# illini-robomaster/irmv_detection

Measured on AMD Instinct MI355X. Metric: end-to-end FPS (preprocess→NMS→PnP) 640×640 YOLOv8n, 1/2/4/8 MI355X, higher is better.
Workload: dtype f16

## Files before the change

### irmv_detection_amd/csrc/engine.cpp

```cpp
#include "engine_internal.hpp"

static thread_local std::string g_err;
int irmv::fail(int code, const std::string &msg) { g_err = msg; return code; }

extern "C" const char *irmv_last_error(void) { return g_err.c_str(); }
extern "C" const char *irmv_version(void)
{
    static char buf[96];
    static std::once_flag once;
    std::call_once(once, [] {
        int v = 0;
        if (hipRuntimeGetVersion(&v) != hipSuccess) v = 0;
        snprintf(buf, sizeof buf, "irmv_hip 0.3 (gfx950; HIP runtime %d)", v);
    });
    return buf;
}
extern "C" int irmv_device_synchronize(int device)
{
    HIP_TRY(hipSetDevice(device));
    HIP_TRY(hipDeviceSynchronize());
    return IRMV_OK;
}
extern "C" int irmv_device_count(int *count)
{
// ... 199 lines not shown
    cfg->bayer_gain_q8[0] = cfg->bayer_gain_q8[1] = cfg->bayer_gain_q8[2] = 256;
}

static EngineSwitches read_switches()
{
    auto set = [](const char *name) { return getenv(name) != nullptr; };
    auto starts = [](const char *name, char c) { const char *v = getenv(name); return v && v[0] == c; };
    auto off = [&](const char *name) { return starts(name, '0'); };
    auto is1 = [&](const char *name) { return starts(name, '1'); };
    EngineSwitches s;
    TuneSwitches &t = s.tune;
    t.untuned = off("IRMV_AUTOTUNE"); t.verbose = set("IRMV_AUTOTUNE_VERBOSE"); t.warn = set("IRMV_TUNE_WARN");
    const char *s2 = getenv("IRMV_FORCE_S2"), *wres = getenv("IRMV_FORCE_WRES");
    t.has_s2 = s2 != nullptr; t.force_s2 = s2 ? s2 : "";
    t.has_wres = wres != nullptr; t.force_wres = wres ? wres : "";
    t.force_pw = set("IRMV_FORCE_PW"); t.force_pwn = set("IRMV_FORCE_PWN"); t.force_cm = set("IRMV_FORCE_CM");
    t.force_w8 = set("IRMV_FORCE_W8"); t.force_nt8 = set("IRMV_FORCE_NT8"); t.force_pf4 = set("IRMV_FORCE_PF4");
    t.no_pw = set("IRMV_NO_PW"); t.no_pwn = set("IRMV_NO_PWN"); t.no_pf2 = set("IRMV_NO_PF2"); t.no_pf4 = set("IRMV_NO_PF4");
    t.no_cm = set("IRMV_NO_CM"); t.no_w8 = set("IRMV_NO_W8"); t.no_nt8 = set("IRMV_NO_NT8"); t.no_wres = set("IRMV_NO_WRES");
    t.no_deep = is1("IRMV_NO_DEEP");
    s.front.fastx = !off("IRMV_FRONT_FASTX"); s.front.direct = !off("IRMV_FRONT_DIRECT"); s.front.tall = !off("IRMV_FRONT_TILE8");
    s.fused_front = !off("IRMV_FUSED_FRONT"); s.fused_c2f = !off("IRMV_FUSED_C2F"); s.bneck64 = !off("IRMV_BNECK64"); s.kpt3 = !off("IRMV_KPT3");
    s.fused_head = !off("IRMV_FUSED_HEAD");
    s.merge_head0 = off("IRMV_MERGE_HEAD0") ? 0 : (is1("IRMV_MERGE_HEAD0") ? 1 : -1);
    s.group_head = !off("IRMV_GROUP_HEAD"); s.group_verbose = set("IRMV_GROUP_VERBOSE"); s.group_force = set("IRMV_GROUP_FORCE");
    if (const char *ns = getenv("IRMV_STREAMS")) { s.has_streams = true; s.streams = atoi(ns); }
    s.numa = !off("IRMV_NUMA");
    s.inline_copies = is1("IRMV_INLINE_COPIES"); s.graph_upload = !off("IRMV_GRAPH_UPLOAD"); s.window_upload = !off("IRMV_WINDOW_UPLOAD");
    if (const char *uk = getenv("IRMV_UPLOAD_KERNEL")) s.upload_kernel_blocks = atoi(uk);
    s.sync_launch = starts("IRMV_SYNC_LAUNCH", 'e') ? 1 : (starts("IRMV_SYNC_LAUNCH", 'g') ? 0 : -1);
    s.split_scan = !off("IRMV_SPLIT_SCAN"); s.emit_scan = !off("IRMV_EMIT_SCAN");
    s.sparse_head = !off("IRMV_SPARSE_HEAD"); s.sparse_branch = !off("IRMV_SPARSE_BRANCH");
    s.sparse_gather = !off("IRMV_SPARSE_GATHER");
    if (const char *gg = getenv("IRMV_SPARSE_GATHER_GRID")) s.gather_grid = atoi(gg);
    s.zero_copy_results = !off("IRMV_ZERO_COPY_RESULTS"); s.post_keys_only = is1("IRMV_POST_KEYS_ONLY");
    s.nms_classwalk = !off("IRMV_NMS_CLASSWALK");
    s.meter_merge = !off("IRMV_METER_MERGE");
    s.nms_prefilter = off("IRMV_NMS_PREFILTER") ? 0 : 1;
    if (const char *pe = getenv("IRMV_NMS_PRE")) { int hi = 0, lo = 0; if (sscanf(pe, "%d,%d", &hi, &lo) == 2 && hi >= 64 && hi <= 512 && lo >= 32 && lo < hi) s.nms_prefilter = hi | (lo << 16); }
    if (const char *st = getenv("IRMV_NMS_STAMPS")) { s.nms_stamps = true; s.nms_stamps_slots = atoi(st); }
    return s;
}

constexpr size_t kCfgSizeV1 = offsetof(irmv_engine_cfg, src_format);
constexpr size_t kCfgSizeV2 = offsetof(irmv_engine_cfg, reserved2);
static_assert(offsetof(irmv_engine_cfg, net_height) < kCfgSizeV2 && kCfgSizeV2 < sizeof(irmv_engine_cfg), "three distinct cfg sizes");
static_assert(offsetof(irmv_engine_cfg, win_width) == offsetof(irmv_engine_cfg, reserved2) + 4 && offsetof(irmv_engine_cfg, win_height) + 2 == sizeof(irmv_engine_cfg),
              "win_width / win_height fill the tail of irmv_engine_cfg");

static irmv_engine_cfg window_view(const irmv_engine_cfg &c)
{
    irmv_engine_cfg v = c;
    if (c.win_width > 0 && c.win_height > 0) { v.src_width = c.win_width; v.src_height = c.win_height; }
    v.win_width = v.win_height = 0;
    return v;
}

int irmv::check_letterbox(const irmv_engine_cfg &c)
{
    int nw, nh;
    scaled_size(c, &nw, &nh);
    if (nw < 1 || nh < 1) return fail(IRMV_ERR_ARG, "letterbox: the scaled frame has no row or no column; use IRMV_RESIZE_STRETCH");
    return IRMV_OK;
}

int irmv::resolve_cfg(const irmv_engine_cfg *cfg_in, irmv_engine_cfg *full)
// ... 668 lines not shown
```

### irmv_detection_amd/csrc/engine_internal.hpp

```cpp
#pragma once
#include <hip/hip_runtime.h>

#include <algorithm>
#include <chrono>
#include <cmath>
#include <cstdio>
#include <cstring>
#include <fstream>
#include <map>
#include <mutex>
#include <set>
#include <memory>
#include <string>
#include <vector>

#include "../../include/irmv_hip.h"
#include "irmv_common.hpp"
#include "numa.hpp"

using namespace irmv;

namespace irmv { int fail(int code, const std::string &msg); }
#define HIP_TRY(expr)                                                                                 \
    do {                                                                                              \
// ... 39 lines not shown
struct DevRange { std::string name; MemTag tag; void *base; size_t bytes; };

struct FrontSwitches { bool fastx = true, direct = true, tall = true; };

struct TuneSwitches {
    bool untuned, verbose, warn;
    bool has_s2, has_wres;
    std::string force_s2, force_wres;
    bool force_pw, force_pwn, force_cm, force_w8, force_nt8, force_pf4;
    bool no_pw, no_pwn, no_pf2, no_pf4, no_cm, no_w8, no_nt8, no_wres, no_deep;
};

struct EngineSwitches {
    TuneSwitches tune{};
    FrontSwitches front;
    bool fused_front = true, fused_c2f = true;
    bool bneck64 = true;
    bool kpt3 = true;
    bool fused_head = true;
    int merge_head0 = -1;
    bool group_head = true;
    bool group_verbose = false;
    bool group_force = false;
    bool has_streams = false; int streams = 0;
    bool numa = true;
    bool inline_copies = false;
    bool graph_upload = true;
    int upload_kernel_blocks = 256;
    bool window_upload = true;
    int sync_launch = -1;
    bool split_scan = true;
    bool emit_scan = true, sparse_head = true, sparse_branch = true;
    bool sparse_gather = true;
    int gather_grid = 0;
    bool zero_copy_results = true;
    bool post_keys_only = false;
    bool nms_classwalk = true;
    int nms_prefilter = 1;
    bool meter_merge = true;
    bool nms_stamps = false; int nms_stamps_slots = 0;
};

enum OpKind { OP_PRE, OP_CONV0, OP_CONV, OP_POOL, OP_NMS, OP_LIGHT, OP_FRONT, OP_C2F2, OP_C2F32, OP_DW, OP_SHUF, OP_SCAN, OP_BNECK, OP_KPT3, OP_BOXG, OP_DEMOSAIC, OP_CROP, OP_METER, OP_YAW, OP_PATCH, OP_NUMBER };

struct Op {
    OpKind kind;
    std::string layer;
    ConvCfg cfg{};
    ConvCfg cfg_one{};
    char kname_one[48] = {0};
    SegRef s0, s1;
    int Hin = 0, Win = 0, Hout = 0, Wout = 0, cin = 0, cout = 0, cout_pad = 0, ksteps = 0;
    int out_t = -1, out_coff = 0, res_t = -1, res_coff = 0;
    half_t *w_packed = nullptr;
    half_t *w_k16 = nullptr;
    half_t *w_lds[4] = {nullptr, nullptr, nullptr, nullptr};
    float *bias = nullptr;
    double flops = 0, bytes = 0;
    double w_bytes = 0;
    double out_bytes = 0;
    bool pair = false;
    int level = -1;
    char kname[48] = {0};
    int sub[4] = {-1, -1, -1, -1};
    int mode = 0;
    bool shortcut = false;
    int fuse_next = -1;
    bool fused_away = false;
    int group = -1;
    int bneck = -1;
    int kpt3 = -1;
    int boxg = -1;
    bool gated_first = false;
    int tune_fuse[2] = {-1, -1};
};

enum StepKind { STEP_BATCH, STEP_ONE, STEP_MATERIALIZE, STEP_POST };

struct Launch {
    int op = -1, group = -1;
    bool cfg_one = false;
    bool fused = false;
    unsigned scan = 0;
    bool keys_only = false;
    bool sparse = false;
    int gate = 0;
    bool cand_list = false;
    bool once = false;
    std::string name, layer;
    double flops = 0, bytes = 0, launch_bytes = 0;
};

struct Step {
    StepKind kind;
    int first, count;
    int tile_frame = -1;
    bool crop_pinned = false;
    bool tiled() const { return tile_frame >= 0; }
    bool dev_records() const { return tiled(); }
    int bayer_first() const { return tiled() ? tile_frame : first; }
    int bayer_count() const { return tiled() ? 1 : count; }
    bool operator<(const Step &o) const { return std::tie(first, count, kind, tile_frame, crop_pinned) < std::tie(o.first, o.count, o.kind, o.tile_frame, o.crop_pinned); }
};

struct GraphKey {
    Step step;
    bool upload;
    int view;
    bool operator<(const GraphKey &o) const { return std::tie(upload, view, step) < std::tie(o.upload, o.view, o.step); }
};

enum UploadForm {
    UP_NONE,
    UP_PINNED_CROP,
    UP_KERNEL,
    UP_COPY,
    UP_BANDS,
};
struct Upload { UploadForm form = UP_NONE; int first = 0, count = 0; };

// ... 255 lines not shown
```

### irmv_detection_amd/csrc/engine_plan.cpp

```cpp
#include "engine_internal.hpp"

static bool is_cls_final_carrier(const Op &op) { return op.fuse_next >= 0 && op.level >= 0 && op.layer.rfind("model.22.cv3.", 0) == 0; }

void irmv::finalize_head_fusion(irmv_engine *e)
{
    for (Op &op : e->ops) {
        if (op.fuse_next < 0) continue;
        const bool k16 = op.cfg.cin16 && !op.cfg.lds && !op.cfg_one.lds && !op.cfg.deep && !op.cfg_one.deep && op.cfg.nt == 1 && op.cfg_one.nt == 1 && e->ops[op.fuse_next].w_k16;
        const bool ok = k16 || (op.cfg.lds && op.cfg.nt == 4 && op.cfg_one.lds && op.cfg_one.nt == 4);
        if (!ok) { op.fuse_next = -1; continue; }
        e->ops[op.fuse_next].fused_away = true;
        e->lazy_tensors.insert(e->tensors[op.out_t].name);
        const size_t l = strlen(op.kname), l1 = strlen(op.kname_one);
        snprintf(op.kname + l, sizeof op.kname - l, "+1x1");
        snprintf(op.kname_one + l1, sizeof op.kname_one - l1, "+1x1");
    }
    int fused = 0;
    for (const Op &op : e->ops) fused += is_cls_final_carrier(op);
    e->emit_scan = e->sw.split_scan && fused == 3 && e->sw.emit_scan;
    e->sparse_head = e->emit_scan && e->cand_bits && e->sw.sparse_head;
    e->sparse_branch = e->sparse_head && e->sw.sparse_branch;
}

static bool is_box_final_carrier(const Op &op) { return op.fuse_next >= 0 && op.level >= 0 && op.layer.rfind("model.22.cv2.", 0) == 0; }

static void sparse_head_plan(irmv_engine *e, std::vector<Launch> &plan)
{
    int last_cls = -1;
    bool lvl_cls[3] = {false, false, false};
    for (size_t i = 0; i < plan.size(); i++)
        if (plan[i].scan && plan[i].group < 0) { last_cls = (int)i; lvl_cls[e->ops[plan[i].op].level] = true; }
    auto box_carrier = [&](const Launch &l) {
        const Op &op = e->ops[l.op];
        return l.group < 0 && l.fused && op.kind == OP_CONV && is_box_final_carrier(op) && op.level < 3 && lvl_cls[op.level];
    };
    std::vector<char> first_conv(plan.size(), 0);
    if (e->sparse_branch)
        for (size_t i = 0; i < plan.size(); i++) {
            const Launch &f = plan[i];
            const Op &fo = e->ops[f.op];
            if (f.group >= 0 || f.fused || f.scan || fo.kind != OP_CONV || !(f.cfg_one ? fo.cfg_one : fo.cfg).wr || fo.res_t >= 0) continue;
            int carrier = -1;
            for (size_t j = i + 1; j < plan.size(); j++) {
                const Op &co = e->ops[plan[j].op];
                if (box_carrier(plan[j]) && co.level == fo.level && co.s0.t == fo.out_t && co.s1.C == 0 && co.s0.coff == fo.out_coff && co.Hin == fo.Hout && co.Win == fo.Wout) carrier = plan[j].op;
            }
            bool other = false;
            for (int k = 0; k < (int)e->ops.size(); k++) {
                const Op &o = e->ops[k];
                if (k == carrier || k == f.op) continue;
                other = other || o.s0.t == fo.out_t || o.s1.t == fo.out_t || o.res_t == fo.out_t || o.out_t == fo.out_t;
            }
            first_conv[i] = carrier >= 0 && !other;
        }
    std::vector<Launch> out, moved;
    bool listed = false;
    for (size_t i = 0; i < plan.size(); i++) {
        Launch &l = plan[i];
        Op &op = e->ops[l.op];
        const bool boxg = op.kind == OP_BOXG;
        if (boxg) {
            l.sparse = true;
            l.cand_list = !listed;
            listed = true;
        }
        if (l.scan) {
            if (l.group < 0) l.bytes -= e->ops[op.fuse_next].out_bytes;
            else for (size_t m = 0; m < e->head_groups[l.group].members.size(); m++)
                if (l.scan >> m & 1u) l.bytes -= e->ops[e->ops[e->head_groups[l.group].members[m]].fuse_next].out_bytes;
        }
        const bool cls_first = op.level >= 0 && op.level < 3 && lvl_cls[op.level];
        const bool box = box_carrier(l);
        const bool kpt = op.kind == OP_KPT3 && cls_first && (int)i > last_cls;
        if (box || kpt) {
            l.sparse = true;
            l.bytes -= box ? e->ops[op.fuse_next].out_bytes : op.out_bytes;
            if (e->sparse_branch) l.gate = 1;
        }
        if (first_conv[i]) {
            l.gate = 2;
            op.gated_first = true;
            e->lazy_tensors.insert(e->tensors[op.out_t].name);
        }
        if ((box || first_conv[i] || boxg) && (int)i < last_cls) moved.push_back(l); else out.push_back(l);
        if ((int)i == last_cls) { out.insert(out.end(), moved.begin(), moved.end()); moved.clear(); }
    }
    plan.swap(out);
}

static bool box_gathers(const irmv_engine *e, const Op &g, bool one)
// ... 122 lines not shown
```

### irmv_detection_amd/csrc/engine_step.cpp

```cpp
#include "engine_internal.hpp"

void irmv::fill_conv_args(const irmv_engine *e, const Op &op, int first, int count, ConvArgs &a, bool fused)
{
    a = ConvArgs{};
    auto seg = [&](const SegRef &s) {
        ConvSeg cs{nullptr, 0, 0, 0};
        if (s.t < 0 || s.C == 0) return cs;
        const Tensor &t = e->tensors[s.t];
        cs.p = static_cast<const half_t *>(t.slot(first)) + s.coff;
        cs.ld = t.C;
        cs.C = s.C;
        cs.shift = s.shift;
        return cs;
    };
    a.s0 = seg(op.s0);
    a.s1 = seg(op.s1);
    a.Hin = op.Hin; a.Win = op.Win; a.Hout = op.Hout; a.Wout = op.Wout;
    a.M = count * op.Hout * op.Wout;
    a.Cin = op.cin;
    a.w = op.w_packed;
    a.bias = op.bias;
    const Tensor &ot = e->tensors[op.out_t];
    a.out = static_cast<char *>(ot.slot(first)) + (size_t)op.out_coff * ot.esize();
    a.out_ld = ot.C;
// ... 225 lines not shown
}

static Kpt3Args kpt3_args(const irmv_engine *e, const Op &op, const Launch &l, int first, const PostArgs &pa)
{
    const Op &o0 = e->ops[op.sub[0]], &o1 = e->ops[op.sub[1]], &o2 = e->ops[op.sub[2]];
    const Tensor &xt = e->tensors[o0.s0.t], &ht = e->tensors[o2.out_t];
    Kpt3Args a{};
    a.x = static_cast<const half_t *>(xt.slot(first)) + o0.s0.coff; a.x_ld = xt.C;
    a.H = op.Hin; a.W = op.Win;
    a.tiles_x = (op.Win + kKpt3Tile - 1) / kKpt3Tile; a.tiles_y = (op.Hin + kKpt3Tile - 1) / kKpt3Tile;
    a.w1 = o0.w_lds[0]; a.b1 = o0.bias;
    a.w2 = o1.w_packed; a.b2 = o1.bias;
    a.w3 = o2.w_k16; a.b3 = o2.bias;
    a.out = static_cast<float *>(ht.slot(first)) + o2.out_coff; a.out_ld = ht.C;
    if (l.sparse) { a.cand_bits = pa.cand_bits; a.cand_words = pa.cand_words; a.abase = e->lvl_base[op.level]; a.tile_gate = l.gate; }
    return a;
}

static CandListArgs cand_list_args(const irmv_engine *e, int first, const PostArgs &pa)
{
    CandListArgs a{};
    a.cand_bits = pa.cand_bits; a.cand_words = pa.cand_words;
    const size_t S = (size_t)e->cfg.num_slots;
    for (int l = 0; l < 3; l++) { a.abase[l] = e->lvl_base[l]; a.hw[l] = e->lvl_hw[l]; }
    for (const Op &op : e->ops)
        if (op.kind == OP_BOXG) {
            const int l = op.level;
            a.list[l] = e->boxg_list + (size_t)e->lvl_base[l] * S + (size_t)first * e->lvl_hw[l];
            a.count[l] = e->boxg_count + (size_t)l * S + first;
        }
    return a;
}

static BoxGatherArgs boxg_args(const irmv_engine *e, const Op &op, int first, const PostArgs &pa)
{
    const Op &o0 = e->ops[op.sub[0]], &o1 = e->ops[op.sub[1]], &o2 = e->ops[op.sub[2]];
    const Tensor &xt = e->tensors[o0.s0.t], &ht = e->tensors[o2.out_t];
    const CandListArgs c = cand_list_args(e, first, pa);
    BoxGatherArgs a{};
    a.x = static_cast<const half_t *>(xt.slot(first)) + o0.s0.coff; a.x_ld = xt.C;
    a.H = op.Hin; a.W = op.Win;
    a.w0 = o0.w_lds[2]; a.b0 = o0.bias;
    a.w1 = o1.w_lds[2]; a.b1 = o1.bias;
    a.w2 = o2.w_packed; a.b2 = o2.bias;
    a.out = static_cast<float *>(ht.slot(first)) + o2.out_coff; a.out_ld = ht.C;
    a.list = c.list[op.level]; a.count = c.count[op.level];
    return a;
}

static DwArgs dw_args(const irmv_engine *e, const Op &op, int first)
{
    DwArgs a;
    const Tensor &xt = e->tensors[op.s0.t], &ot = e->tensors[op.out_t];
    a.x = static_cast<const half_t *>(xt.slot(first)) + op.s0.coff; a.x_ld = xt.C;
    a.y = static_cast<half_t *>(ot.slot(first)) + op.out_coff; a.y_ld = ot.C;
    a.w = op.w_packed; a.b = op.bias;
    a.Hin = op.Hin; a.Win = op.Win; a.Hout = op.Hout; a.Wout = op.Wout; a.C = op.cout; a.stride = op.cfg.stride;
    return a;
}

static ShufArgs shuf_args(const irmv_engine *e, const Op &op, int first, int count)
{
    ShufArgs a;
    const Tensor &at = e->tensors[op.s0.t], &bt = e->tensors[op.s1.t], &ot = e->tensors[op.out_t];
    a.a = static_cast<const half_t *>(at.slot(first)) + op.s0.coff; a.a_ld = at.C;
    a.b = static_cast<const half_t *>(bt.slot(first)) + op.s1.coff; a.b_ld = bt.C;
    a.out = static_cast<half_t *>(ot.slot(first)); a.out_ld = ot.C;
    a.bc = op.s0.C;
    a.pixels = (size_t)count * op.Hin * op.Win;
    return a;
}

static Conv0Args conv0_args(const irmv_engine *e, const Op &op, int first, int count)
{
    Conv0Args a;
    a.x = static_cast<const half_t *>(e->tensors[op.s0.t].slot(first));
    a.y = static_cast<half_t *>(e->tensors[op.out_t].slot(first));
    a.w = e->conv0_w; a.b = e->conv0_b; a.net_w = e->cfg.net_size; a.net_h = e->cfg.net_height; a.batch = count;
    return a;
// ... 14 lines not shown
    ConvWeights w[kMultiMax];
    const int n = (int)g.members.size();
    for (int k = 0; k < n; k++) {
        const Op &op = e->ops[g.members[k]];
        fill_conv_args(e, op, first, 1, a[k], true);
        if (scan >> k & 1u) scan_args_for(e, op, *pa, a[k]);
        w[k] = conv_weights(op);
    }
    return g.family == 0 ? launch_conv_lds_multi(g.nt, a, w, n, 1, s) : launch_conv_direct_multi(g.cfg, a, n, s);
}

int irmv::launch_op(irmv_engine *e, const View &v, const Launch &l, const Step &t, const PostArgs &pa, unsigned scan, hipStream_t s)
{
    const Op &op = e->ops[l.op];
    const int first = t.first, count = t.count;
    switch (op.kind) {
    case OP_DEMOSAIC: launch_bayer(e, t.bayer_first(), t.bayer_count(), s); break;
    case OP_CROP: launch_crop(e, t, s); break;
    case OP_METER: launch_meter(e, v, t, s); break;
    case OP_YAW: launch_yaw(e, t, pa, s); break;
    case OP_PATCH: launch_patch(e, v, t, pa, s); break;
    case OP_NUMBER: launch_number(e, t, pa, s); break;
    case OP_PRE: launch_preprocess(pre_args(e, v, op, first), count, s); break;
    case OP_FRONT: if (!launch_front(front_args(e, v, op, first), count, s)) return fail(IRMV_ERR_HIP, "fused front kernel: LDS request refused"); break;
    case OP_C2F2: launch_c2f2(c2f2_args(e, op, first), count, s); break;
    case OP_C2F32: if (!launch_c2f32(op.mode, op.shortcut, c2f32_args(e, op, first, count), count, s)) return fail(IRMV_ERR_ARG, "no fused C2f kernel for " + op.layer); break;
    case OP_BNECK:
        if (!launch_bneck64(op.mode, op.sub[2] >= 0 ? e->ops[op.sub[2]].ksteps : 6, op.shortcut, bneck_args(e, op, first), count, s)) return fail(IRMV_ERR_ARG, "no fused bottleneck kernel for " + op.layer);
        break;
    case OP_KPT3: if (!launch_kpt3(kpt3_args(e, op, l, first, pa), op.cin, count, s)) return fail(IRMV_ERR_ARG, "no fused keypoint-branch kernel for " + op.layer); break;
    case OP_BOXG:
        if (!pa.cand_bits) return fail(IRMV_ERR_ARG, "a box gather launch needs the sparse head's bitmap: " + op.layer);
        if (l.cand_list) launch_cand_list(cand_list_args(e, first, pa), count, s);
        if (!launch_box_gather(boxg_args(e, op, first, pa), op.cin, count, e->sw.gather_grid > 0 ? e->sw.gather_grid : e->num_cus, s)) return fail(IRMV_ERR_ARG, "no box gather kernel for " + op.layer);
        break;
    case OP_DW: launch_dwconv3x3(dw_args(e, op, first), count, s); break;
    case OP_SHUF: launch_shuffle_cat(shuf_args(e, op, first, count), s); break;
    case OP_CONV0: launch_conv0(conv0_args(e, op, first, count), s); break;
    case OP_POOL: { const Tensor &t = e->tensors[op.out_t]; launch_sppf_pool(static_cast<half_t *>(t.slot(first)), count, t.H, t.W, t.C / 4, s); break; }
    case OP_CONV: {
        if (l.group >= 0) {
            if (!launch_head_group(e, e->head_groups[l.group], first, &pa, scan, s)) return fail(IRMV_ERR_ARG, "grouped launch refused: " + l.name);
            break;
        }
        ConvArgs a;
        fill_conv_args(e, op, first, count, a, l.fused);
        if (scan) scan_args_for(e, op, pa, a);
        if (l.sparse || l.gate) { a.cand_bits = pa.cand_bits; a.cand_words = pa.cand_words; a.scan_abase = e->lvl_base[op.level]; a.tile_gate = l.gate; }
        if (!run_conv(op, l.cfg_one ? op.cfg_one : op.cfg, a, count, s)) return fail(IRMV_ERR_ARG, std::string("no conv kernel for ") + op.kname + " (" + op.layer + ")");
        break;
    }
    case OP_SCAN: launch_scan_decode(pa, count, s); break;
    case OP_NMS: { PostArgs pn = pa; pn.keys_only = l.keys_only ? 1 : 0; launch_nms_pnp(pn, count, s); break; }
    case OP_LIGHT: launch_light_extract(light_args(e, v, first), e->cfg.max_det, count, s); break;
    }
    HIP_TRY(hipGetLastError());
    return IRMV_OK;
}

int irmv::enqueue_step(irmv_engine *e, const Step &t, hipStream_t s, int reps, const std::vector<hipEvent_t> *ev)
{
    const View &v = view_of(e, t.first);
    const std::vector<Launch> &plan = v.plans[t.kind];
    const PostArgs pa = post_args(e, v, t);
    PostArgs mute = pa;
    mute.cls = e->cls_dev + 1;
    for (size_t i = 0; i < plan.size(); i++) {
// ... 361 lines not shown
```

### irmv_detection_amd/csrc/irmv_common.hpp

```cpp
#pragma once

#include <hip/hip_runtime.h>

#include <cstdint>
#include <cstdlib>

namespace irmv {

typedef _Float16 half_t;
typedef _Float16 half8 __attribute__((ext_vector_type(8)));
typedef _Float16 half4 __attribute__((ext_vector_type(4)));
typedef float f32x4 __attribute__((ext_vector_type(4)));

constexpr float kActScale = 1.44269504088896341f;
constexpr float kActUnscale = 0.693147180559945309f;
typedef unsigned int u32x4_t __attribute__((ext_vector_type(4)));
__device__ __forceinline__ float silu_rcp(float y) { return __builtin_amdgcn_rcpf(1.0f + __builtin_amdgcn_exp2f(-y)); }
__device__ __forceinline__ unsigned int silu_pack2(float y0, float y1)
{
    const float r0 = silu_rcp(y0), r1 = silu_rcp(y1);
    unsigned int o;
    asm("v_fma_mixlo_f16 %0, %1, %2, 0" : "=v"(o) : "v"(y0), "v"(r0));
    asm("v_fma_mixhi_f16 %0, %1, %2, 0" : "+v"(o) : "v"(y1), "v"(r1));
    return o;
// ... 204 lines not shown
    const half_t *w3;
    const float *b3;
    float *out;
    int out_ld;
    const unsigned int *cand_bits;
    int cand_words, abase;
    int tile_gate;
};
bool kpt3_eligible(int cin);
bool launch_kpt3(const Kpt3Args &a, int cin, int batch, hipStream_t s);

struct CandListArgs {
    const unsigned int *cand_bits;
    int cand_words;
    int abase[3], hw[3];
    int *list[3];
    int *count[3];
};
void launch_cand_list(const CandListArgs &a, int batch, hipStream_t s);
struct BoxGatherArgs {
    const half_t *x;
    int x_ld;
    int H, W;
    const half_t *w0;
    const float *b0;
    const half_t *w1;
    const float *b1;
    const half_t *w2;
    const float *b2;
    float *out;
    int out_ld;
    const int *list;
    const int *count;
};
bool box_gather_eligible(int cin);
bool launch_box_gather(const BoxGatherArgs &a, int cin, int batch, int grid, hipStream_t s);

constexpr int kMaxClasses = 16;
struct ClassTable {
    float min_thr;
    int32_t pad_[3];
    float thr[kMaxClasses];
    int32_t plate[kMaxClasses];
};

struct ConvArgs {
    ConvSeg s0, s1;
    int Hin, Win;
    int Hout, Wout;
    int M;
    int Cin;
    const half_t *w;
    const float *bias;
    void *out;
    int out_ld;
    const half_t *res;
    int res_ld;
    int cout_pad;
    int ksteps;
    int pair;
    const half_t *w2;
    const float *bias2;
    float *out2;
    int out2_ld, n2;
    unsigned long long *scan_keys;
    int *scan_counts;
// ... 370 lines not shown
```

### irmv_detection_amd/csrc/k_boxg.hip

```cpp
#include "irmv_common.hpp"

#include <mutex>

namespace irmv {

namespace {
constexpr int GNG = 2;
constexpr int GNT = GNG * 192;
constexpr int GSLAB = 9 * 4 * 64;
constexpr int GWPT = GSLAB / GNT;
constexpr int GROW = 16 * 128;
constexpr int GMID = 9 * GROW;
constexpr int GMAXB = 1024;
constexpr size_t GWLDS = (size_t)2 * GSLAB * 16;
constexpr size_t GLDS = GWLDS + (size_t)GNG * GMID + (size_t)GMAXB * 4;
static_assert(GSLAB % GNT == 0, "every thread stages the same number of slab pieces");
static_assert(GLDS <= 160 * 1024, "a CU's LDS");
}

__global__ __launch_bounds__(256) void cand_list_kernel(CandListArgs a)
{
    __shared__ int s_n[3];
    const int img = blockIdx.x, tid = threadIdx.x;
    if (tid < 3) s_n[tid] = 0;
    __syncthreads();
    const int A = a.abase[2] + a.hw[2];
    for (int wd = tid; wd < a.cand_words; wd += 256) {
        unsigned int w = a.cand_bits[(size_t)img * a.cand_words + wd];
        while (w) {
            const int an = wd * 32 + __builtin_ctz(w);
            w &= w - 1u;
            const int lv = an >= a.abase[2] ? 2 : (an >= a.abase[1] ? 1 : 0);
            if (an < A && a.list[lv]) a.list[lv][(size_t)img * a.hw[lv] + atomicAdd(&s_n[lv], 1)] = an - a.abase[lv];
        }
    }
    __syncthreads();
    if (tid < 3 && a.count[tid]) a.count[tid][img] = s_n[tid];
}

void launch_cand_list(const CandListArgs &a, int batch, hipStream_t s)
{
    hipLaunchKernelGGL(cand_list_kernel, dim3(batch), dim3(256), 0, s, a);
}

template <int STEPS>
__global__ __launch_bounds__(GNT) void box_gather_kernel(BoxGatherArgs a, int batch)
{
    extern __shared__ __attribute__((aligned(16))) uint8_t smem[];
    half8 *s_w2 = reinterpret_cast<half8 *>(smem);
    uint8_t *s_mid = smem + GWLDS;
    int *s_pre = reinterpret_cast<int *>(smem + GWLDS + (size_t)GNG * GMID);
    constexpr int CH1 = 2 * STEPS, NCH = CH1 + 2;
    const int tid = threadIdx.x, lane = tid & 63;
    const int wave = __builtin_amdgcn_readfirstlane(tid >> 6);
    const int sub = wave / 3, row = wave - sub * 3;
    const int g = lane >> 4, r = lane & 15;
    const int H = a.H, W = a.W, HW = H * W;

    if (wave == 0) {
        int carry = 0;
        for (int base = 0; base < batch; base += 64) {
            const int i = base + lane;
            int v = i < batch ? min(max(a.count[i], 0), HW) : 0;
#pragma unroll
            for (int d = 1; d < 64; d <<= 1) {
                const int t = __shfl_up(v, d);
                if (lane >= d) v += t;
            }
            v += carry;
            if (i < batch) s_pre[i] = v;
            carry = __shfl(v, 63);
        }
    }
    __syncthreads();
    const int n = s_pre[batch - 1];
    if ((int)blockIdx.x * (GNG * 16) >= n) return;

    const int img_stride = HW * a.x_ld * 2;
    const auto rs_x = __builtin_amdgcn_make_buffer_rsrc(const_cast<half_t *>(a.x), 0, batch * img_stride, 0x00020000);
    const half8 *w0 = reinterpret_cast<const half8 *>(a.w0), *w1 = reinterpret_cast<const half8 *>(a.w1);
    half8 rw[GWPT];
    auto fetch_slab = [&](int k) {
        const half8 *src = k < CH1 ? w0 + (size_t)k * GSLAB : w1 + (size_t)(k - CH1) * GSLAB;
#pragma unroll
        for (int i = 0; i < GWPT; i++) rw[i] = src[tid + i * GNT];
    };
    static_assert(NCH % 2 == 0, "slab k of every pass lies in buffer k & 1");
    auto stage_slab = [&](int k) {
        half8 *s_w = s_w2 + (k & 1) * GSLAB;
#pragma unroll
        for (int i = 0; i < GWPT; i++) s_w[tid + i * GNT] = rw[i];
        fetch_slab(k + 1 < NCH ? k + 1 : 0);
        __syncthreads();
        return s_w;
    };
    auto bias_of = [&](const float *b, int nt) { return *reinterpret_cast<const f32x4 *>(b + (nt >> 1) * 32 + g * 8 + (nt & 1) * 4); };
    auto slot = [&](int c) { return r * 128 + ((c ^ (r & 7) ^ (r >> 3)) & 7) * 16; };
    uint8_t *mid = s_mid + (size_t)sub * GMID;
    fetch_slab(0);

    for (int pass = blockIdx.x; pass * (GNG * 16) < n; pass += gridDim.x) {
        const int k = pass * (GNG * 16) + sub * 16 + r;
        const bool valid = k < n;
        const int kk = valid ? k : n - 1;
        int lo = 0, hi = batch - 1;
        while (lo < hi) {
            const int m = (lo + hi) >> 1;
            if (s_pre[m] > kk) hi = m; else lo = m + 1;
        }
        const int img = lo;
        const int ent = kk - (img > 0 ? s_pre[img - 1] : 0);
        const int p = min(max(a.list[(size_t)img * HW + ent], 0), HW - 1);
        const int cy = p / W, cx = p - cy * W;

        f32x4 acc[3][4];
        int src[3][5];
        bool inmap[3];
#pragma unroll
        for (int kh = 0; kh < 3; kh++)
#pragma unroll
            for (int j = 0; j < 5; j++) {
                const int iy = cy + row - 2 + kh, ix = cx - 2 + j;
                const bool in = valid && (unsigned)iy < (unsigned)H && (unsigned)ix < (unsigned)W;
                src[kh][j] = in ? (((img * H + iy) * W + ix) * a.x_ld + g * 8) * 2 : 0x7fffffff;
            }
#pragma unroll
        for (int i = 0; i < 3; i++) {
            inmap[i] = (unsigned)(cy + row - 1) < (unsigned)H && (unsigned)(cx + i - 1) < (unsigned)W;
#pragma unroll
            for (int nt = 0; nt < 4; nt++) acc[i][nt] = bias_of(a.b0, nt);
        }

        for (int c = 0; c < CH1; c++) {
            half8 in[3][5];
#pragma unroll
            for (int kh = 0; kh < 3; kh++)
#pragma unroll
                for (int j = 0; j < 5; j++) in[kh][j] = __builtin_bit_cast(half8, __builtin_amdgcn_raw_buffer_load_b128(rs_x, src[kh][j], c * 64, 0));
            const half8 *s_w = stage_slab(c);
#pragma unroll
            for (int tap = 0; tap < 9; tap++) {
                const int kh = tap / 3, kw = tap - kh * 3;
                half8 A[4];
#pragma unroll
                for (int nt = 0; nt < 4; nt++) A[nt] = s_w[(tap * 4 + nt) * 64 + lane];
#pragma unroll
                for (int i = 0; i < 3; i++)
#pragma unroll
                    for (int nt = 0; nt < 4; nt++) acc[i][nt] = __builtin_amdgcn_mfma_f32_16x16x32_f16(A[nt], in[kh][i + kw], acc[i][nt], 0, 0, 0);
            }
        }
#pragma unroll
        for (int i = 0; i < 3; i++)
#pragma unroll
            for (int u = 0; u < 2; u++) {
                half8 o = silu_pack8(acc[i][2 * u][0], acc[i][2 * u][1], acc[i][2 * u][2], acc[i][2 * u][3],
                                     acc[i][2 * u + 1][0], acc[i][2 * u + 1][1], acc[i][2 * u + 1][2], acc[i][2 * u + 1][3]);
                if (!inmap[i]) o = (half8){0, 0, 0, 0, 0, 0, 0, 0};
                *reinterpret_cast<half8 *>(mid + (row * 3 + i) * GROW + slot(u * 4 + g)) = o;
            }

        f32x4 acc2[4] = {bias_of(a.b1, 0), bias_of(a.b1, 1), bias_of(a.b1, 2), bias_of(a.b1, 3)};
        for (int u = 0; u < 2; u++) {
            const half8 *s_w = stage_slab(CH1 + u);
            if (row == 0) {
#pragma unroll
                for (int tap = 0; tap < 9; tap++) {
                    half8 A[4];
#pragma unroll
                    for (int nt = 0; nt < 4; nt++) A[nt] = s_w[(tap * 4 + nt) * 64 + lane];
                    const half8 B = *reinterpret_cast<const half8 *>(mid + tap * GROW + slot(u * 4 + g));
#pragma unroll
                    for (int nt = 0; nt < 4; nt++) acc2[nt] = __builtin_amdgcn_mfma_f32_16x16x32_f16(A[nt], B, acc2[nt], 0, 0, 0);
                }
            }
        }
        if (row == 0) {
#pragma unroll
            for (int u = 0; u < 2; u++)
                *reinterpret_cast<half8 *>(mid + slot(u * 4 + g)) = silu_pack8(acc2[2 * u][0], acc2[2 * u][1], acc2[2 * u][2], acc2[2 * u][3],
                                                                               acc2[2 * u + 1][0], acc2[2 * u + 1][1], acc2[2 * u + 1][2], acc2[2 * u + 1][3]);
        }
        __syncthreads();

        if (row == 1) {
            const half8 *w2 = reinterpret_cast<const half8 *>(a.w2) + lane;
            const half8 B0 = *reinterpret_cast<const half8 *>(mid + slot(g)), B1 = *reinterpret_cast<const half8 *>(mid + slot(4 + g));
            float *orow = a.out + ((size_t)img * HW + p) * a.out_ld;
#pragma unroll
            for (int t2 = 0; t2 < 4; t2++) {
                f32x4 c2 = (f32x4){0.f, 0.f, 0.f, 0.f};
                c2 = __builtin_amdgcn_mfma_f32_16x16x32_f16(w2[(t2 * 2 + 0) * 64], B0, c2, 0, 0, 0);
                c2 = __builtin_amdgcn_mfma_f32_16x16x32_f16(w2[(t2 * 2 + 1) * 64], B1, c2, 0, 0, 0);
                const int co = t2 * 16 + g * 4;
                const f32x4 b2 = *reinterpret_cast<const f32x4 *>(a.b2 + co);
                const f32x4 v2 = (f32x4){c2[0] * kActUnscale + b2[0], c2[1] * kActUnscale + b2[1], c2[2] * kActUnscale + b2[2], c2[3] * kActUnscale + b2[3]};
                if (valid) *reinterpret_cast<f32x4 *>(orow + co) = v2;
            }
        }
    }
}

bool box_gather_eligible(int cin) { return cin == 64 || cin == 128 || cin == 256; }

bool launch_box_gather(const BoxGatherArgs &a, int cin, int batch, int grid, hipStream_t s)
{
    if (batch < 1 || batch > GMAXB || grid < 1) return false;
    static std::mutex mu;
    static unsigned long long done[3] = {0, 0, 0};
    auto go = [&](auto kernel, unsigned long long &mask) {
        int dev = 0;
        (void)hipGetDevice(&dev);
        {
            std::lock_guard<std::mutex> lk(mu);
            if (!(mask >> (dev & 63) & 1ull)) {
                (void)hipFuncSetAttribute(reinterpret_cast<const void *>(kernel), hipFuncAttributeMaxDynamicSharedMemorySize, (int)GLDS);
                mask |= 1ull << (dev & 63);
            }
        }
        hipLaunchKernelGGL(kernel, dim3(grid), dim3(GNT), GLDS, s, a, batch);
    };
    switch (cin) {
    case 64: go(box_gather_kernel<1>, done[0]); return true;
    case 128: go(box_gather_kernel<2>, done[1]); return true;
    case 256: go(box_gather_kernel<4>, done[2]); return true;
    default: return false;
    }
}

}
```

Measured before the change: 64860.

## Fuse keypoint head into sparse box-gather kernel as an extra wave per group

```diff
diff --git a/irmv_detection_amd/csrc/engine.cpp b/irmv_detection_amd/csrc/engine.cpp
--- a/irmv_detection_amd/csrc/engine.cpp
+++ b/irmv_detection_amd/csrc/engine.cpp
@@ -255,6 +255,7 @@
     s.split_scan = !off("IRMV_SPLIT_SCAN"); s.emit_scan = !off("IRMV_EMIT_SCAN");
     s.sparse_head = !off("IRMV_SPARSE_HEAD"); s.sparse_branch = !off("IRMV_SPARSE_BRANCH");
     s.sparse_gather = !off("IRMV_SPARSE_GATHER");
+    s.gather_kpt = !off("IRMV_GATHER_KPT"); s.kpt3_named = is1("IRMV_KPT3");
     if (const char *gg = getenv("IRMV_SPARSE_GATHER_GRID")) s.gather_grid = atoi(gg);
     s.zero_copy_results = !off("IRMV_ZERO_COPY_RESULTS"); s.post_keys_only = is1("IRMV_POST_KEYS_ONLY");
     s.nms_classwalk = !off("IRMV_NMS_CLASSWALK");
diff --git a/irmv_detection_amd/csrc/engine_internal.hpp b/irmv_detection_amd/csrc/engine_internal.hpp
--- a/irmv_detection_amd/csrc/engine_internal.hpp
+++ b/irmv_detection_amd/csrc/engine_internal.hpp
@@ -95,6 +95,8 @@
     bool split_scan = true;
     bool emit_scan = true, sparse_head = true, sparse_branch = true;
     bool sparse_gather = true;
+    bool gather_kpt = true;
+    bool kpt3_named = false;
     int gather_grid = 0;
     bool zero_copy_results = true;
     bool post_keys_only = false;
@@ -149,6 +151,7 @@
     bool sparse = false;
     int gate = 0;
     bool cand_list = false;
+    int kpt = -1;
     bool once = false;
     std::string name, layer;
     double flops = 0, bytes = 0, launch_bytes = 0;
diff --git a/irmv_detection_amd/csrc/engine_plan.cpp b/irmv_detection_amd/csrc/engine_plan.cpp
--- a/irmv_detection_amd/csrc/engine_plan.cpp
+++ b/irmv_detection_amd/csrc/engine_plan.cpp
@@ -53,9 +53,24 @@
             }
             first_conv[i] = carrier >= 0 && !other;
         }
+    std::vector<char> rides(plan.size(), 0);
+    if (e->sw.gather_kpt && !e->sw.kpt3_named)
+        for (size_t i = 0; i < plan.size(); i++) {
+            const Op &ko = e->ops[plan[i].op];
+            if (ko.kind != OP_KPT3 || ko.level < 0 || ko.level >= 3 || !lvl_cls[ko.level] || (int)i <= last_cls) continue;
+            for (size_t j = 0; j < plan.size() && !rides[i]; j++) {
+                const Op &go = e->ops[plan[j].op];
+                if (go.kind != OP_BOXG || go.level != ko.level) continue;
+                const Op &k0 = e->ops[ko.sub[0]], &g0 = e->ops[go.sub[0]];
+                if (k0.s0.t != g0.s0.t || k0.s0.coff != g0.s0.coff || k0.cin != g0.cin || ko.Hin != go.Hin || ko.Win != go.Win) continue;
+                plan[j].kpt = plan[i].op;
+                rides[i] = 1;
+            }
+        }
     std::vector<Launch> out, moved;
     bool listed = false;
     for (size_t i = 0; i < plan.size(); i++) {
+        if (rides[i]) continue;
         Launch &l = plan[i];
         Op &op = e->ops[l.op];
         const bool boxg = op.kind == OP_BOXG;
diff --git a/irmv_detection_amd/csrc/engine_step.cpp b/irmv_detection_amd/csrc/engine_step.cpp
--- a/irmv_detection_amd/csrc/engine_step.cpp
+++ b/irmv_detection_amd/csrc/engine_step.cpp
@@ -281,7 +281,7 @@
     return a;
 }
 
-static BoxGatherArgs boxg_args(const irmv_engine *e, const Op &op, int first, const PostArgs &pa)
+static BoxGatherArgs boxg_args(const irmv_engine *e, const Op &op, const Launch &l, int first, const PostArgs &pa)
 {
     const Op &o0 = e->ops[op.sub[0]], &o1 = e->ops[op.sub[1]], &o2 = e->ops[op.sub[2]];
     const Tensor &xt = e->tensors[o0.s0.t], &ht = e->tensors[o2.out_t];
@@ -294,6 +294,15 @@
     a.w2 = o2.w_packed; a.b2 = o2.bias;
     a.out = static_cast<float *>(ht.slot(first)) + o2.out_coff; a.out_ld = ht.C;
     a.list = c.list[op.level]; a.count = c.count[op.level];
+    if (l.kpt >= 0) {
+        const Op &k = e->ops[l.kpt];
+        const Op &k0 = e->ops[k.sub[0]], &k1 = e->ops[k.sub[1]], &k2 = e->ops[k.sub[2]];
+        const Tensor &kt = e->tensors[k2.out_t];
+        a.kw0 = k0.w_lds[0]; a.kb0 = k0.bias;
+        a.kw1 = k1.w_packed; a.kb1 = k1.bias;
+        a.kw2 = k2.w_k16; a.kb2 = k2.bias;
+        a.kout = static_cast<float *>(kt.slot(first)) + k2.out_coff; a.kout_ld = kt.C;
+    }
     return a;
 }
 
@@ -374,7 +383,7 @@
     case OP_BOXG:
         if (!pa.cand_bits) return fail(IRMV_ERR_ARG, "a box gather launch needs the sparse head's bitmap: " + op.layer);
         if (l.cand_list) launch_cand_list(cand_list_args(e, first, pa), count, s);
-        if (!launch_box_gather(boxg_args(e, op, first, pa), op.cin, count, e->sw.gather_grid > 0 ? e->sw.gather_grid : e->num_cus, s)) return fail(IRMV_ERR_ARG, "no box gather kernel for " + op.layer);
+        if (!launch_box_gather(boxg_args(e, op, l, first, pa), op.cin, count, e->sw.gather_grid > 0 ? e->sw.gather_grid : e->num_cus, s)) return fail(IRMV_ERR_ARG, "no box gather kernel for " + op.layer);
         break;
     case OP_DW: launch_dwconv3x3(dw_args(e, op, first), count, s); break;
     case OP_SHUF: launch_shuffle_cat(shuf_args(e, op, first, count), s); break;
diff --git a/irmv_detection_amd/csrc/irmv_common.hpp b/irmv_detection_amd/csrc/irmv_common.hpp
--- a/irmv_detection_amd/csrc/irmv_common.hpp
+++ b/irmv_detection_amd/csrc/irmv_common.hpp
@@ -260,6 +260,14 @@
     int out_ld;
     const int *list;
     const int *count;
+    const half_t *kw0;
+    const float *kb0;
+    const half_t *kw1;
+    const float *kb1;
+    const half_t *kw2;
+    const float *kb2;
+    float *kout;
+    int kout_ld;
 };
 bool box_gather_eligible(int cin);
 bool launch_box_gather(const BoxGatherArgs &a, int cin, int batch, int grid, hipStream_t s);
diff --git a/irmv_detection_amd/csrc/k_boxg.hip b/irmv_detection_amd/csrc/k_boxg.hip
--- a/irmv_detection_amd/csrc/k_boxg.hip
+++ b/irmv_detection_amd/csrc/k_boxg.hip
@@ -7,6 +7,7 @@
 namespace {
 constexpr int GNG = 2;
 constexpr int GNT = GNG * 192;
+constexpr int GNTK = GNG * 256;
 constexpr int GSLAB = 9 * 4 * 64;
 constexpr int GWPT = GSLAB / GNT;
 constexpr int GROW = 16 * 128;
@@ -14,8 +15,11 @@
 constexpr int GMAXB = 1024;
 constexpr size_t GWLDS = (size_t)2 * GSLAB * 16;
 constexpr size_t GLDS = GWLDS + (size_t)GNG * GMID + (size_t)GMAXB * 4;
+constexpr int KROW = 16 * 32;
+constexpr int KMID = 10 * KROW;
+constexpr size_t GLDSK = GLDS + (size_t)GNG * KMID;
 static_assert(GSLAB % GNT == 0, "every thread stages the same number of slab pieces");
-static_assert(GLDS <= 160 * 1024, "a CU's LDS");
+static_assert(GLDSK <= 160 * 1024, "a CU's LDS");
 }
 
 __global__ __launch_bounds__(256) void cand_list_kernel(CandListArgs a)
@@ -43,17 +47,19 @@
     hipLaunchKernelGGL(cand_list_kernel, dim3(batch), dim3(256), 0, s, a);
 }
 
-template <int STEPS>
-__global__ __launch_bounds__(GNT) void box_gather_kernel(BoxGatherArgs a, int batch)
+template <int STEPS, bool KPT>
+__global__ __launch_bounds__(KPT ? GNTK : GNT) void box_gather_kernel(BoxGatherArgs a, int batch)
 {
     extern __shared__ __attribute__((aligned(16))) uint8_t smem[];
     half8 *s_w2 = reinterpret_cast<half8 *>(smem);
     uint8_t *s_mid = smem + GWLDS;
     int *s_pre = reinterpret_cast<int *>(smem + GWLDS + (size_t)GNG * GMID);
     constexpr int CH1 = 2 * STEPS, NCH = CH1 + 2;
-    const int tid = threadIdx.x, lane = tid & 63;
-    const int wave = __builtin_amdgcn_readfirstlane(tid >> 6);
-    const int sub = wave / 3, row = wave - sub * 3;
+    constexpr int NW = KPT ? 4 : 3;
+    const int lane = threadIdx.x & 63;
+    const int wave = __builtin_amdgcn_readfirstlane(threadIdx.x >> 6);
+    const int sub = wave / NW, row = wave - sub * NW;
+    const int tid = (int)threadIdx.x - (KPT ? sub * 64 : 0);
     const int g = lane >> 4, r = lane & 15;
     const int H = a.H, W = a.W, HW = H * W;
 
@@ -97,40 +103,169 @@
     auto bias_of = [&](const float *b, int nt) { return *reinterpret_cast<const f32x4 *>(b + (nt >> 1) * 32 + g * 8 + (nt & 1) * 4); };
     auto slot = [&](int c) { return r * 128 + ((c ^ (r & 7) ^ (r >> 3)) & 7) * 16; };
     uint8_t *mid = s_mid + (size_t)sub * GMID;
-    fetch_slab(0);
-
-    for (int pass = blockIdx.x; pass * (GNG * 16) < n; pass += gridDim.x) {
-        const int k = pass * (GNG * 16) + sub * 16 + r;
-        const bool valid = k < n;
+    auto candidate = [&](int pass, int slot, bool &valid, int &img, int &p) {
+        const int k = pass * (GNG * 16) + sub * 16 + slot;
+        valid = k < n;
         const int kk = valid ? k : n - 1;
         int lo = 0, hi = batch - 1;
         while (lo < hi) {
             const int m = (lo + hi) >> 1;
             if (s_pre[m] > kk) hi = m; else lo = m + 1;
         }
-        const int img = lo;
+        img = lo;
         const int ent = kk - (img > 0 ? s_pre[img - 1] : 0);
-        const int p = min(max(a.list[(size_t)img * HW + ent], 0), HW - 1);
+        p = min(max(a.list[(size_t)img * HW + ent], 0), HW - 1);
+    };
+
+    const int from = (r * 4 + g) * 4;
+    auto to_mfma_lanes = [&](half8 (&row)[5]) {
+#pragma unroll
+        for (int j = 0; j < 5; j++) {
+            u32x4_t v = __builtin_bit_cast(u32x4_t, row[j]);
+#pragma unroll
+            for (int d = 0; d < 4; d++) v[d] = (unsigned int)__builtin_amdgcn_ds_bpermute(from, (int)v[d]);
+            row[j] = __builtin_bit_cast(half8, v);
+        }
+    };
+
+    if constexpr (KPT) {
+        if (row == 3) {
+            uint8_t *kp = smem + GLDS + (size_t)sub * KMID;
+            const auto rs_w = __builtin_amdgcn_make_buffer_rsrc(const_cast<half_t *>(a.kw0), 0, CH1 * 9 * 1024, 0x00020000);
+            auto load_w = [&](int k) { return __builtin_bit_cast(half8, __builtin_amdgcn_raw_buffer_load_b128(rs_w, lane * 16, k * 1024, 0)); };
+            half8 A[9];
+#pragma unroll
+            for (int tap = 0; tap < 9; tap++) A[tap] = load_w(tap);
+            const int tap_lo = g >> 1;
+            for (int pass = blockIdx.x; pass * (GNG * 16) < n; pass += gridDim.x) {
+                bool valid;
+                int img, p;
+                candidate(pass, lane >> 2, valid, img, p);
+                const int cy = p / W, cx = p - cy * W;
+                unsigned int inside = 0u;
+#pragma unroll
+                for (int i = 0; i < 5; i++)
+#pragma unroll
+                    for (int j = 0; j < 5; j++)
+                        inside |= (valid && (unsigned)(cy - 2 + i) < (unsigned)H && (unsigned)(cx - 2 + j) < (unsigned)W ? 1u : 0u) << (i * 5 + j);
+                const int corner = (((img * H + cy - 2) * W + cx - 2) * a.x_ld + (lane & 3) * 8) * 2;
+                const unsigned int inside_m = (unsigned int)__builtin_amdgcn_ds_bpermute(from, (int)inside);
+                const int orow = __builtin_amdgcn_ds_bpermute(from, img * HW + p);
+                auto src = [&](int i, int j) { return (inside >> (i * 5 + j) & 1u) ? corner + (i * W + j) * a.x_ld * 2 : 0x7fffffff; };
+                const f32x4 kb0 = *reinterpret_cast<const f32x4 *>(a.kb0 + g * 4);
+                f32x4 acc[9];
+#pragma unroll
+                for (int q = 0; q < 9; q++) acc[q] = kb0;
+                auto load_row = [&](half8 (&dst)[5], int i, int c) {
+#pragma unroll
+                    for (int j = 0; j < 5; j++) dst[j] = __builtin_bit_cast(half8, __builtin_amdgcn_raw_buffer_load_b128(rs_x, src(i, j), c * 64, 0));
+                };
+                half8 in[5][5];
+#pragma unroll
+                for (int i = 0; i < 5; i++) load_row(in[i], i, 0);
+                __builtin_amdgcn_sched_barrier(0);
+                to_mfma_lanes(in[0]);
+                for (int c = 0; c < CH1; c++) {
+                    const bool more = c + 1 < CH1;
+                    const int cn = more ? c + 1 : 0;
+                    __syncthreads();
+#pragma unroll
+                    for (int i = 0; i < 5; i++) {
+                        if (i < 4) to_mfma_lanes(in[i + 1]);
+                        else if (more) to_mfma_lanes(in[0]);
+#pragma unroll
+                        for (int py = 0; py < 3; py++) {
+                            const int kh = i - py;
+                            if (kh < 0 || kh > 2) continue;
+#pragma unroll
+                            for (int kw = 0; kw < 3; kw++)
+#pragma unroll
+                                for (int px = 0; px < 3; px++)
+                                    acc[py * 3 + px] = __builtin_amdgcn_mfma_f32_16x16x32_f16(A[kh * 3 + kw], in[i][px + kw], acc[py * 3 + px], 0, 0, 0);
+                        }
+                        __builtin_amdgcn_sched_barrier(0);
+                        if (more) load_row(in[i], i, c + 1);
+                        if (i >= 2) {
+#pragma unroll
+                            for (int kw = 0; kw < 3; kw++) A[(i - 2) * 3 + kw] = load_w(cn * 9 + (i - 2) * 3 + kw);
+                        }
+                        __builtin_amdgcn_sched_barrier(0);
+                    }
+                }
+#pragma unroll
+                for (int q = 0; q < 9; q++) {
+                    const int py = q / 3, px = q - py * 3;
+                    half4 o = silu_pack4(acc[q][0], acc[q][1], acc[q][2], acc[q][3]);
+                    if (!(inside_m >> ((py + 1) * 5 + px + 1) & 1u)) o = (half4){0, 0, 0, 0};
+                    *reinterpret_cast<half4 *>(kp + q * KROW + r * 32 + g * 8) = o;
+                }
+                __syncthreads();
+                {
+                    const half8 *w2p = reinterpret_cast<const half8 *>(a.kw1);
+                    f32x4 c1 = *reinterpret_cast<const f32x4 *>(a.kb1 + g * 4);
+                    half8 A2[5], B2[5];
+#pragma unroll
+                    for (int ks = 0; ks < 5; ks++) A2[ks] = w2p[ks * 64 + (ks == 4 ? (lane & 31) : lane)];
+                    if (g >= 2) A2[4] = (half8){0, 0, 0, 0, 0, 0, 0, 0};
+#pragma unroll
+                    for (int ks = 0; ks < 5; ks++) {
+                        const int tap = 2 * ks + tap_lo;
+                        const half8 q = *reinterpret_cast<const half8 *>(kp + (tap < 9 ? tap : 0) * KROW + r * 32 + (g & 1) * 16);
+                        B2[ks] = tap < 9 ? q : (half8){0, 0, 0, 0, 0, 0, 0, 0};
+                    }
+#pragma unroll
+                    for (int ks = 0; ks < 5; ks++) c1 = __builtin_amdgcn_mfma_f32_16x16x32_f16(A2[ks], B2[ks], c1, 0, 0, 0);
+                    *reinterpret_cast<half4 *>(kp + 9 * KROW + r * 32 + g * 8) = silu_pack4(c1[0], c1[1], c1[2], c1[3]);
+                }
+                {
+                    const half4 w3f = *reinterpret_cast<const half4 *>(a.kw2 + lane * 4);
+                    int g4 = g * 4;
+                    asm volatile("" : "+v"(g4));
+                    const f32x4 b3 = *reinterpret_cast<const f32x4 *>(a.kb2 + g4);
+                    __syncthreads();
+                    __syncthreads();
+                    const half4 B = *reinterpret_cast<const half4 *>(kp + 9 * KROW + r * 32 + g * 8);
+                    const f32x4 c2 = __builtin_amdgcn_mfma_f32_16x16x16f16(w3f, B, (f32x4){0.f, 0.f, 0.f, 0.f}, 0, 0, 0);
+                    const f32x4 v2 = (f32x4){c2[0] * kActUnscale + b3[0], c2[1] * kActUnscale + b3[1], c2[2] * kActUnscale + b3[2], c2[3] * kActUnscale + b3[3]};
+                    if (inside_m >> 12 & 1u) *reinterpret_cast<f32x4 *>(a.kout + (size_t)orow * a.kout_ld + g4) = v2;
+                }
+            }
+            return;
+        }
+    }
+    fetch_slab(0);
+
+    for (int pass = blockIdx.x; pass * (GNG * 16) < n; pass += gridDim.x) {
+        bool valid;
+        int img, p;
+        candidate(pass, lane >> 2, valid, img, p);
         const int cy = p / W, cx = p - cy * W;
 
         f32x4 acc[3][4];
         int src[3][5];
-        bool inmap[3];
 #pragma unroll
         for (int kh = 0; kh < 3; kh++)
 #pragma unroll
             for (int j = 0; j < 5; j++) {
                 const int iy = cy + row - 2 + kh, ix = cx - 2 + j;
                 const bool in = valid && (unsigned)iy < (unsigned)H && (unsigned)ix < (unsigned)W;
-                src[kh][j] = in ? (((img * H + iy) * W + ix) * a.x_ld + g * 8) * 2 : 0x7fffffff;
-            }
+                src[kh][j] = in ? (((img * H + iy) * W + ix) * a.x_ld + (lane & 3) * 8) * 2 : 0x7fffffff;
+            }
+        int mine = valid ? 8 : 0;
+#pragma unroll
+        for (int i = 0; i < 3; i++) mine |= ((unsigned)(cy + row - 1) < (unsigned)H && (unsigned)(cx + i - 1) < (unsigned)W ? 1 : 0) << i;
+        mine = __builtin_amdgcn_ds_bpermute(from, mine);
+        const int head_row = __builtin_amdgcn_ds_bpermute(from, img * HW + p);
+        valid = (mine & 8) != 0;
+        bool inmap[3];
 #pragma unroll
         for (int i = 0; i < 3; i++) {
-            inmap[i] = (unsigned)(cy + row - 1) < (unsigned)H && (unsigned)(cx + i - 1) < (unsigned)W;
+            inmap[i] = (mine >> i & 1) != 0;
 #pragma unroll
             for (int nt = 0; nt < 4; nt++) acc[i][nt] = bias_of(a.b0, nt);
         }
 
+#pragma unroll 1
         for (int c = 0; c < CH1; c++) {
             half8 in[3][5];
 #pragma unroll
@@ -138,6 +273,8 @@
 #pragma unroll
                 for (int j = 0; j < 5; j++) in[kh][j] = __builtin_bit_cast(half8, __builtin_amdgcn_raw_buffer_load_b128(rs_x, src[kh][j], c * 64, 0));
             const half8 *s_w = stage_slab(c);
+#pragma unroll
+            for (int kh = 0; kh < 3; kh++) to_mfma_lanes(in[kh]);
 #pragma unroll
             for (int tap = 0; tap < 9; tap++) {
                 const int kh = tap / 3, kw = tap - kh * 3;
@@ -186,7 +323,7 @@
         if (row == 1) {
             const half8 *w2 = reinterpret_cast<const half8 *>(a.w2) + lane;
             const half8 B0 = *reinterpret_cast<const half8 *>(mid + slot(g)), B1 = *reinterpret_cast<const half8 *>(mid + slot(4 + g));
-            float *orow = a.out + ((size_t)img * HW + p) * a.out_ld;
+            float *orow = a.out + (size_t)head_row * a.out_ld;
 #pragma unroll
             for (int t2 = 0; t2 < 4; t2++) {
                 f32x4 c2 = (f32x4){0.f, 0.f, 0.f, 0.f};
@@ -207,23 +344,25 @@
 {
     if (batch < 1 || batch > GMAXB || grid < 1) return false;
     static std::mutex mu;
-    static unsigned long long done[3] = {0, 0, 0};
+    static unsigned long long done[6] = {0, 0, 0, 0, 0, 0};
+    const bool kpt = a.kw0 != nullptr;
+    const size_t lds = kpt ? GLDSK : GLDS;
     auto go = [&](auto kernel, unsigned long long &mask) {
         int dev = 0;
         (void)hipGetDevice(&dev);
         {
             std::lock_guard<std::mutex> lk(mu);
             if (!(mask >> (dev & 63) & 1ull)) {
-                (void)hipFuncSetAttribute(reinterpret_cast<const void *>(kernel), hipFuncAttributeMaxDynamicSharedMemorySize, (int)GLDS);
+                (void)hipFuncSetAttribute(reinterpret_cast<const void *>(kernel), hipFuncAttributeMaxDynamicSharedMemorySize, (int)lds);
                 mask |= 1ull << (dev & 63);
             }
         }
-        hipLaunchKernelGGL(kernel, dim3(grid), dim3(GNT), GLDS, s, a, batch);
+        hipLaunchKernelGGL(kernel, dim3(grid), dim3(kpt ? GNTK : GNT), lds, s, a, batch);
     };
     switch (cin) {
-    case 64: go(box_gather_kernel<1>, done[0]); return true;
-    case 128: go(box_gather_kernel<2>, done[1]); return true;
-    case 256: go(box_gather_kernel<4>, done[2]); return true;
+    case 64: if (kpt) go(box_gather_kernel<1, true>, done[3]); else go(box_gather_kernel<1, false>, done[0]); return true;
+    case 128: if (kpt) go(box_gather_kernel<2, true>, done[4]); else go(box_gather_kernel<2, false>, done[1]); return true;
+    case 256: if (kpt) go(box_gather_kernel<4, true>, done[5]); else go(box_gather_kernel<4, false>, done[2]); return true;
     default: return false;
     }
 }
```

After: 66640 (median of 6 runs). 1.03x the previous value.
